# aclyde11/molecular-VAE

Measured on AMD Instinct MI355X. Metric: molecules/s (ELBO fwd+bwd+step), higher is better.
Workload: dtype bf16

## Files before the change

include/mvae.h:

```cpp
#ifndef MVAE_H_
#define MVAE_H_

#include <stddef.h>
#include <stdint.h>

#ifdef __cplusplus
extern "C" {
#endif

#define MVAE_ABI_VERSION 12

#define MVAE_OK 0
#define MVAE_ERR_INVALID (-1)
#define MVAE_ERR_WORKSPACE (-2)
#define MVAE_ERR_UNSUPPORTED (-3)

#define MVAE_F32 0
#define MVAE_BF16 1
#define MVAE_F32X3 2

#define MVAE_ACT_NONE 0
#define MVAE_ACT_SELU 1
#define MVAE_ACT_RELU 2

// ... 102 lines not shown
  int cell, dtype, layers, T, B, H;
  const void* w_hhT[MVAE_MAX_LAYERS]; int64_t ldw_hhT[MVAE_MAX_LAYERS];
  const void* w_ihT[MVAE_MAX_LAYERS]; int64_t ldw_ihT[MVAE_MAX_LAYERS];
  const int32_t* lengths;
  const float* dy; int64_t dy_ld;
  const void* dy_a; int64_t dy_a_ld; const void* dy_w; int64_t dy_w_ld; int dy_k;
  const float* dh_last[MVAE_MAX_LAYERS];
  const void* hs[MVAE_MAX_LAYERS]; int64_t ldh;
  const void* h0[MVAE_MAX_LAYERS]; int64_t ldh0;
  const void* cs[MVAE_MAX_LAYERS];
  const void* gates[MVAE_MAX_LAYERS];
  void* dG[MVAE_MAX_LAYERS]; int64_t ldg;
  void* dGh[MVAE_MAX_LAYERS];
  float* dstate[MVAE_MAX_LAYERS];
  float* dh0[MVAE_MAX_LAYERS];
  void* split_ws; size_t split_ws_bytes;
  const uint8_t* drop_mask[MVAE_MAX_LAYERS];
  float drop_p; uint32_t drop_seed;
  void* persist_ws; size_t persist_ws_bytes;
  float* poison;
  int no_spin;
} mvae_rnn_bwd_desc;

int mvae_rnn_bwd(const mvae_rnn_bwd_desc* d, void* stream, const void** status_out);
size_t mvae_rnn_bwd_persist_workspace(const mvae_rnn_bwd_desc* d);
size_t mvae_rnn_bwd_workspace(const mvae_rnn_bwd_desc* d);

int mvae_rowsum(int dtype, int R, int C, const void* X, int64_t ldx, float* out, int accumulate, void* stream);
int mvae_timesum(int dtype, int T, int B, int W, const void* X, float* out, void* stream);
size_t mvae_colsum_workspace(int M, int N);
int mvae_colsum(int M, int N, const float* X, int64_t ldx, float* out, void* ws, size_t ws_bytes, void* stream);
size_t mvae_colsum_t_workspace(int M, int N);
int mvae_colsum_t(int dtype, int M, int N, const void* X, int64_t ldx, float* out, void* ws, size_t ws_bytes, void* stream);

int mvae_conv1d_pack_weights(int Cin, int Cout, int k, const float* w , int ldx, float* wp, int ldo, float* wq,
                             void* stream);
size_t mvae_conv1d_selu_fwd_workspace(int B, int W, int ldx, int Cout, int k);
int mvae_conv1d_selu_fwd(int B, int W, int ldx, int64_t x_bs, int Cout, int k, const float* x, const float* wp, const float* bias,
                         float* y, int64_t ldy, void* ws, size_t ws_bytes, void* stream);
size_t mvae_conv1d_selu_bwd_workspace(int B, int W, int Cin, int ldx, int Cout, int ldo, int k);
int mvae_conv1d_act_fwd(int act, int B, int W, int ldx, int64_t x_bs, int Cout, int k, const float* x, const float* wp, const float* bias,
                        float* y, int64_t ldy, void* ws, size_t ws_bytes, void* stream);
#define MVAE_CONV_BWD_X3 0x100
int mvae_conv1d_act_bwd(int act, int B, int W, int Cin, int ldx, int64_t x_bs, int Cout, int ldo, int k, const float* dy, const float* y,
                        const float* x, const float* wq, float* dzp, float* dw, float* db, float* dx, int64_t lddx,
                        void* ws, size_t ws_bytes, void* stream);
int mvae_conv1d_dw_problem(int B, int W, int Cin, int ldx, int64_t x_bs, int Cout, int ldo, int k, const float* dzp, const float* x, float* dwp,
                           float* db, int x3, mvae_gemm_tn_f32_problem* out);
int mvae_conv1d_unpack_dw(int Cin, int Cout, int k, const float* dwp, int ldx, float* dw, void* stream);
int mvae_conv1d_selu_bwd(int B, int W, int Cin, int ldx, int64_t x_bs, int Cout, int ldo, int k, const float* dy, const float* y,
                         const float* x, const float* wq, float* dzp, float* dw, float* db, float* dx, int64_t lddx,
                         void* ws, size_t ws_bytes, void* stream);

int mvae_selu_bwd(int64_t n, float* dy, const float* y, void* stream);

int mvae_lambda_fwd(int B, int o, const float* mulv, const float* eps, float scale, uint32_t seed, uint64_t offset, float* eps_out,
                    float* z, float* mu, float* logvar, void* stream);
int mvae_normal_fill(int64_t n, float scale, uint32_t seed, uint64_t offset, float* out, void* stream);
void mvae_normal_words(uint32_t seed, uint64_t counter, uint32_t* words2);
int mvae_lambda_bwd(int B, int o, const float* mulv, const float* eps, const float* dz, const float* dmu,
                    const float* dlogvar, float* dmulv, void* stream);

int mvae_softmax_tb_fwd(int B, int L, int C, const float* logits, int64_t ldl, float* recon, void* stream);
int mvae_softmax_tb_bwd(int dtype, int B, int L, int C, const float* recon, const float* drecon,
                        void* dl, int64_t ldd, void* dlT, int64_t ldT, void* stream);

// ... 255 lines not shown
```

molecular-vae_amd/_lib.py:

```python
import ctypes as C
import os
import weakref

import torch

_HERE = os.path.dirname(os.path.abspath(__file__))
LIB_PATH = ((os.environ.get("MVAE_LIB") if os.environ.get("MVAE_TUNING", "0") not in ("", "0") else None)
            or os.path.join(_HERE, "libmvae_hip.so"))

ABI_VERSION = 12
MVAE_F32, MVAE_BF16, MVAE_F32X3 = 0, 1, 2
CONV_BWD_X3 = 0x100
ACT_NONE, ACT_SELU, ACT_RELU = 0, 1, 2
CELL_LSTM, CELL_GRU = 0, 1
MAX_LAYERS = 8

_vp, _i, _i64, _f, _sz, _u32 = C.c_void_p, C.c_int, C.c_int64, C.c_float, C.c_size_t, C.c_uint32


class RnnFwdDesc(C.Structure):
    _fields_ = [("cell", _i), ("dtype", _i), ("layers", _i), ("T", _i), ("B", _i), ("H", _i), ("in0", _i),
                ("x0", _vp), ("x0_ld", _i64), ("add0", _vp), ("add0_tstride", _i64),
                ("add_table", _vp), ("add_index", _vp), ("add_index_ld", _i64), ("add_table_rows", _i),
                ("w_ih", _vp * MAX_LAYERS), ("ldw_ih", _i64 * MAX_LAYERS),
# ... 59 lines not shown
    "mvae_cast_transpose": (_i, [_i, _i, _i, _i, _vp, _i64, _vp, _i64, _vp, _i64, _vp]),
    "mvae_pack_job_blocks": (_i, [C.POINTER(PackJob)]),
    "mvae_pack_multi": (_i, [_i, _vp, _i, _vp]),
    "mvae_permute021": (_i, [_i, _i, _i, _vp, _vp, _vp]),
    "mvae_gather_rows_tb": (_i, [_vp, _i, _i, _i, _vp, _i, _vp, _vp, _vp]),
    "mvae_scatter_rows_tb": (_i, [_i, _vp, _i, _i, _i, _vp, _i64, _i, _vp, _vp, _sz, _vp]),
    "mvae_scatter_rows_tb_workspace": (_sz, [_i, _i, _i, _i]),
    "mvae_onehot_tb": (_i, [_vp, _i, _i, _i, _vp, _i64, _vp]),
    "mvae_onehot_f32": (_i, [_vp, _i64, _i, _vp, _i64, _vp]),
    "mvae_rnn_fwd": (_i, [C.POINTER(RnnFwdDesc), _vp, C.POINTER(_vp)]),
    "mvae_rnn_fwd_persist_workspace": (_sz, [C.POINTER(RnnFwdDesc)]),
    "mvae_dropout_keep": (_i, [C.c_uint32, C.c_uint32, _f]),
    "mvae_gemm_tn_f32_colsum": (_i, [_i, _i, _i, _vp, _i64, _vp, _i64, _vp, _i64, _i, _vp, _i, _vp, _sz, _vp]),
    "mvae_gemm_tn_colsum_supported": (_i, [_i, _i, _i]),
    "mvae_gemm_tn_grouped_supported": (_i, [_i, _i, _i64, _i64, _i64]),
    "mvae_gemm_tn_grouped_workspace": (_sz, [_i, C.POINTER(GemmTnProblem)]),
    "mvae_gemm_tn_grouped": (_i, [_i, C.POINTER(GemmTnProblem), _vp, _sz, _vp]),
    "mvae_gemm_tn_grouped_capped": (_i, [_i, C.POINTER(GemmTnProblem), _i, _vp, _sz, _vp]),
    "mvae_gemm_tn_f32_multi_workspace": (_sz, [_i, C.POINTER(GemmTnF32Problem)]),
    "mvae_gemm_tn_f32_multi": (_i, [_i, C.POINTER(GemmTnF32Problem), _vp, _sz, _vp]),
    "mvae_conv1d_dw_problem": (_i, [_i, _i, _i, _i, _i64, _i, _i, _i, _vp, _vp, _vp, _vp, _i, C.POINTER(GemmTnF32Problem)]),
    "mvae_conv1d_unpack_dw": (_i, [_i, _i, _i, _vp, _i, _vp, _vp]),
    "mvae_gemm_tn_colsum_workspace": (_sz, [_i, _i, _i]),
    "mvae_gemm_tn_colsum": (_i, [_i, _i, _i, _vp, _i64, _vp, _i64, _vp, _i64, _i, _vp, _i, _vp, _sz, _vp]),
    "mvae_rnn_bwd": (_i, [C.POINTER(RnnBwdDesc), _vp, C.POINTER(_vp)]),
    "mvae_rnn_bwd_workspace": (_sz, [C.POINTER(RnnBwdDesc)]),
    "mvae_rnn_bwd_persist_workspace": (_sz, [C.POINTER(RnnBwdDesc)]),
    "mvae_rowsum": (_i, [_i, _i, _i, _vp, _i64, _vp, _i, _vp]),
    "mvae_timesum": (_i, [_i, _i, _i, _i, _vp, _vp, _vp]),
    "mvae_colsum_workspace": (_sz, [_i, _i]),
    "mvae_colsum": (_i, [_i, _i, _vp, _i64, _vp, _vp, _sz, _vp]),
    "mvae_colsum_t_workspace": (_sz, [_i, _i]),
    "mvae_colsum_t": (_i, [_i, _i, _i, _vp, _i64, _vp, _vp, _sz, _vp]),
    "mvae_conv1d_pack_weights": (_i, [_i, _i, _i, _vp, _i, _vp, _i, _vp, _vp]),
    "mvae_conv1d_selu_fwd_workspace": (_sz, [_i, _i, _i, _i, _i]),
    "mvae_conv1d_selu_fwd": (_i, [_i, _i, _i, _i64, _i, _i, _vp, _vp, _vp, _vp, _i64, _vp, _sz, _vp]),
    "mvae_conv1d_selu_bwd_workspace": (_sz, [_i, _i, _i, _i, _i, _i, _i]),
    "mvae_conv1d_selu_bwd": (_i, [_i, _i, _i, _i, _i64, _i, _i, _i, _vp, _vp, _vp, _vp, _vp, _vp, _vp, _vp, _i64, _vp, _sz, _vp]),
    "mvae_conv1d_act_fwd": (_i, [_i, _i, _i, _i, _i64, _i, _i, _vp, _vp, _vp, _vp, _i64, _vp, _sz, _vp]),
    "mvae_conv1d_act_bwd": (_i, [_i, _i, _i, _i, _i, _i64, _i, _i, _i, _vp, _vp, _vp, _vp, _vp, _vp, _vp, _vp, _i64, _vp, _sz, _vp]),
    "mvae_selu_bwd": (_i, [_i64, _vp, _vp, _vp]),
    "mvae_lambda_fwd": (_i, [_i, _i, _vp, _vp, _f, C.c_uint32, C.c_uint64, _vp, _vp, _vp, _vp, _vp]),
    "mvae_normal_fill": (_i, [_i64, _f, C.c_uint32, C.c_uint64, _vp, _vp]),
    "mvae_normal_words": (None, [C.c_uint32, C.c_uint64, C.POINTER(C.c_uint32)]),
    "mvae_lambda_bwd": (_i, [_i, _i, _vp, _vp, _vp, _vp, _vp, _vp, _vp]),
    "mvae_softmax_tb_fwd": (_i, [_i, _i, _i, _vp, _i64, _vp, _vp]),
    "mvae_softmax_tb_bwd": (_i, [_i, _i, _i, _i, _vp, _vp, _vp, _i64, _vp, _i64, _vp]),
    "mvae_bce_kl_loss_workspace": (_sz, [_i64, _i64]),
    "mvae_bce_kl_loss_fwd": (_i, [_i64, _vp, _vp, _i64, _vp, _vp, _f, _vp, _vp, _sz, _vp]),
    "mvae_bce_kl_loss_bwd": (_i, [_i64, _vp, _vp, _i64, _vp, _vp, _f, _vp, _vp, _vp, _vp, _vp]),
    "mvae_bce_kl_logits_workspace": (_sz, [_i, _i]),
    "mvae_bce_kl_logits_fwd": (_i, [_i, _i, _i, _vp, _i64, _vp, _i64, _vp, _vp, _f, _vp, _vp, _vp, _sz, _vp]),
    "mvae_bce_kl_logits_bwd": (_i, [_i, _i, _i, _i, _vp, _i64, _vp, _i64, _vp, _vp, _f, _vp, _vp, _i64, _vp, _i64, _vp, _vp, _vp]),
    "mvae_expand_indices": (_i, [_vp, _vp, _i, _i, _i, _vp, _vp, _vp]),
    "mvae_moses_collate": (_i, [_vp, _vp, _vp, _i, _i, _i64, _i, _i, _i, _vp, _i64, _vp, _vp, _vp, _vp]),
    "mvae_corpus_index_build": (_i, [_vp, _vp, _i64, _vp, _i64, _vp, _vp]),
    "mvae_corpus_index_probe": (_i, [_vp, _vp, _i64, _vp, _i64, _i, _i, _vp, _i64, _i, _vp, _vp]),
    "mvae_moses_latent_workspace": (_sz, [_i]),
    "mvae_moses_latent_fwd": (_i, [_i, _i, _vp, _vp, _vp, C.c_uint32, C.c_uint64, _vp, _vp, _vp, _vp, _sz, _vp]),
    "mvae_moses_latent_bwd": (_i, [_i, _i, _vp, _vp, _vp, _vp, _vp, _vp, _vp, _vp, _vp]),
    "mvae_moses_latent_fb_workspace": (_sz, [_i, _i]),
    "mvae_moses_latent_fb_fwd": (_i, [_i, _i, _vp, _vp, _vp, C.c_uint32, C.c_uint64, _vp, _f, _vp, _vp, _vp, _vp, _sz, _vp]),
    "mvae_moses_latent_fb_bwd": (_i, [_i, _i, _vp, _vp, _vp, _vp, _vp, _vp, _vp, _f, _vp, _vp, _vp]),
    "mvae_token_dropout": (_i, [_vp, _vp, _i, _i, _i, _f, C.c_uint32, _vp, _vp, _vp, _vp]),
    "mvae_ce_loss_workspace": (_sz, [_i, _i]),
    "mvae_ce_loss_fwd": (_i, [_i, _i, _i, _vp, _i64, _vp, _i, _vp, _vp, _sz, _vp]),
# ... 182 lines not shown
```

molecular-vae_amd/csrc/elementwise.hip:

```cpp
#include "common.hpp"
#include "kernels.hpp"
#include <stdlib.h>

static inline int grid_for(long n, int per_block = 256, int cap = 2048) {
  long b = (n + per_block - 1) / per_block;
  if (b < 1) b = 1;
  if (b > cap) b = cap;
  return (int)b;
}

template <typename TS, typename TD>
__global__ __launch_bounds__(256) void cast_transpose_kernel(int R, int C, const TS* src, long lds_, TD* dst, long ldd, TD* dstT, long ldt) {
  __shared__ float tile[32][33];
  const int c0 = blockIdx.x * 32, r0 = blockIdx.y * 32;
  const int tx = threadIdx.x & 31, ty = threadIdx.x >> 5;
#pragma unroll
  for (int i = 0; i < 4; ++i) {
    const int r = r0 + ty + i * 8, c = c0 + tx;
    float v = 0.f;
    if (r < R && c < C) v = TT<TS>::ld(src + (long)r * lds_ + c);
    tile[ty + i * 8][tx] = v;
    if (dst && r < R && c < ldd) TT<TD>::st(dst + (long)r * ldd + c, v);
  }
  if (!dstT) return;
// ... 89 lines not shown
__global__ __launch_bounds__(256) void scatter_rows_tb_stage1(const int64_t* idx, int B, int L, int nrows, const T* d, long ldd, int W,
                                                              int rpb, int ws_cols, float* partial) {
  extern __shared__ __attribute__((aligned(16))) char smem_raw[];
  float* tab = reinterpret_cast<float*>(smem_raw);
  const long total = (long)B * L;
  const int c_lo = blockIdx.y * ws_cols;
  int c_hi = c_lo + ws_cols; if (c_hi > W) c_hi = W;
  const int wsl = c_hi - c_lo;
  for (int i = threadIdx.x; i < nrows * ws_cols; i += 256) tab[i] = 0.f;
  __syncthreads();
  const long rbeg = (long)blockIdx.x * rpb;
  long rend = rbeg + rpb; if (rend > total) rend = total;
  for (int c = threadIdx.x; c < wsl; c += 256) {
    for (long row0 = rbeg; row0 < rend; row0 += 8) {
      float v[8]; int id[8];
#pragma unroll
      for (int r = 0; r < 8; ++r) {
        const long row = row0 + r;
        if (row < rend) {
          const int t = (int)(row / B), b = (int)(row - (long)t * B);
          long q = idx[(long)b * L + t];
          id[r] = (int)(q < 0 ? 0 : (q >= nrows ? nrows - 1 : q));
          v[r] = TT<T>::ld(d + row * ldd + c_lo + c);
        } else { id[r] = 0; v[r] = 0.f; }
      }
#pragma unroll
      for (int r = 0; r < 8; ++r) tab[id[r] * ws_cols + c] += v[r];
    }
  }
  __syncthreads();
  float* out = partial + (long)blockIdx.x * nrows * W;
  for (int i = threadIdx.x; i < nrows * wsl; i += 256) { const int r = i / wsl, c = i - r * wsl; out[(long)r * W + c_lo + c] = tab[r * ws_cols + c]; }
}
__global__ __launch_bounds__(256) void sum_partials_kernel(const float* partial, int nparts, long n, float* out) {
  __shared__ float red[4][64];
  const int e = threadIdx.x & 63, slot = threadIdx.x >> 6;
  const long i = (long)blockIdx.x * 64 + e;
  float v = 0.f;
  if (i < n) for (int k = slot; k < nparts; k += 4) v += partial[(long)k * n + i];
  red[slot][e] = v;
  __syncthreads();
  if (slot == 0 && i < n) out[i] = (red[0][e] + red[1][e]) + (red[2][e] + red[3][e]);
}

__global__ __launch_bounds__(256) void permute021_kernel(int N, int A, int Bd, const float* in, float* out) {
  const long n = (long)N * A * Bd;
  for (long i = (long)blockIdx.x * 256 + threadIdx.x; i < n; i += (long)gridDim.x * 256) {
    const int a = (int)(i % A); const long nb = i / A; const int b = (int)(nb % Bd); const long nn = nb / Bd;
    out[i] = in[(nn * A + a) * Bd + b];
  }
}

__global__ __launch_bounds__(256) void selu_bwd_kernel(long n, float* dy, const float* y) {
  for (long i = (long)blockIdx.x * 256 + threadIdx.x; i < n; i += (long)gridDim.x * 256) dy[i] *= selu_grad_from_out(y[i]);
}
int launch_selu_bwd(long n, float* dy, const float* y, hipStream_t st) {
  if (n <= 0) return MVAE_OK;
  hipLaunchKernelGGL(selu_bwd_kernel, dim3(grid_for(n)), dim3(256), 0, st, n, dy, y);
  MVAE_CHECK_HIP(hipGetLastError());
  return MVAE_OK;
}

__global__ __launch_bounds__(256) void colsum_stage1_kernel(int M, int N, const float* X, long ldx, int rows_per_chunk, float* partial) {
  __shared__ float red[4][64];
  const int c = blockIdx.x * 64 + (threadIdx.x & 63), g = threadIdx.x >> 6;
  const int r0 = blockIdx.y * rows_per_chunk;
// ... 38 lines not shown
    for (int m = r0 + rs; m < r1; m += 8) {
      float v[8];
      const T* p = X + (long)m * ldx + c0;
      if (n == 8) {
        if constexpr (sizeof(T) == 2) {
          const uint4 u = *reinterpret_cast<const uint4*>(p);
          const uint32_t w[4] = {u.x, u.y, u.z, u.w};
#pragma unroll
          for (int i = 0; i < 4; ++i) { v[2 * i] = __builtin_bit_cast(float, w[i] << 16); v[2 * i + 1] = __builtin_bit_cast(float, w[i] & 0xffff0000u); }
        } else {
          const float4 x0 = *reinterpret_cast<const float4*>(p), x1 = *reinterpret_cast<const float4*>(p + 4);
          v[0] = x0.x; v[1] = x0.y; v[2] = x0.z; v[3] = x0.w; v[4] = x1.x; v[5] = x1.y; v[6] = x1.z; v[7] = x1.w;
        }
      } else {
#pragma unroll
        for (int e = 0; e < 8; ++e) v[e] = (e < n) ? TT<T>::ld(p + e) : 0.f;
      }
#pragma unroll
      for (int e = 0; e < 8; ++e) a[e] += v[e];
    }
  }
#pragma unroll
  for (int e = 0; e < 8; ++e) red[rs][cg * 8 + e] = a[e];
  __syncthreads();
  const int c = blockIdx.x * 256 + threadIdx.x;
  if (c < N) {
    float v = 0.f;
#pragma unroll
    for (int k = 0; k < 8; ++k) v += red[k][threadIdx.x];
    partial[(long)blockIdx.y * N + c] = v;
  }
}
static int colsum_t_chunks(int M) { int c = (M + 511) / 512; if (c > 64) c = 64; if (c < 1) c = 1; return c; }

template <typename T> __device__ __forceinline__ float sum_chunk16(const uint4& v);
template <> __device__ __forceinline__ float sum_chunk16<float>(const uint4& v) {
  return (__builtin_bit_cast(float, v.x) + __builtin_bit_cast(float, v.y)) + (__builtin_bit_cast(float, v.z) + __builtin_bit_cast(float, v.w));
}
template <> __device__ __forceinline__ float sum_chunk16<bf16_t>(const uint4& v) {
  float a = 0.f;
  const uint32_t w[4] = {v.x, v.y, v.z, v.w};
#pragma unroll
  for (int i = 0; i < 4; ++i) a += __builtin_bit_cast(float, w[i] << 16) + __builtin_bit_cast(float, w[i] & 0xffff0000u);
  return a;
}
template <typename T>
__global__ __launch_bounds__(256) void rowsum_kernel(int R, int C, const T* X, long ldx, float* out, int accumulate) {
  constexpr int EPC = TT<T>::EPC;
  const int r = blockIdx.x * 4 + (threadIdx.x >> 6), lane = threadIdx.x & 63;
  if (r >= R) return;
  const T* p = X + (long)r * ldx;
  float v = 0.f;
  int c0 = 0;
  if ((reinterpret_cast<uintptr_t>(p) & 15) == 0) {
    const int nch = C / EPC;
    for (int i = lane; i < nch; i += 64) v += sum_chunk16<T>(*reinterpret_cast<const uint4*>(p + (long)i * EPC));
    c0 = nch * EPC;
  }
  for (int c = c0 + lane; c < C; c += 64) v += TT<T>::ld(p + c);
  v = wave_sum(v);
  if (lane == 0) out[r] = accumulate ? out[r] + v : v;
}
template <typename T>
__global__ __launch_bounds__(256) void timesum_kernel(int T_, long BW, const T* X, float* out) {
  for (long i = (long)blockIdx.x * 256 + threadIdx.x; i < BW; i += (long)gridDim.x * 256) {
    float v = 0.f;
// ... 1012 lines not shown
}

int mvae_pack_job_blocks(const mvae_pack_job* j) {
  if (!j || j->R < 1 || j->C < 1) return 0;
  if (j->kind == 1) return (int)(((long)j->R * j->C + 1023) / 1024);
  return ((j->C + 31) / 32) * ((j->R + 31) / 32);
}
int mvae_pack_multi(int njobs, const mvae_pack_job* jobs_device, int total_blocks, void* stream) {
  if (njobs < 1 || !jobs_device || total_blocks < 1) return MVAE_ERR_INVALID;
  hipLaunchKernelGGL(pack_multi_kernel, dim3((unsigned)total_blocks), dim3(256), 0, (hipStream_t)stream, njobs, jobs_device);
  MVAE_CHECK_HIP(hipGetLastError());
  return MVAE_OK;
}

int mvae_permute021(int N, int A, int Bd, const float* in, float* out, void* stream) {
  if (!in || !out || N < 1 || A < 1 || Bd < 1) return MVAE_ERR_INVALID;
  hipLaunchKernelGGL(permute021_kernel, dim3(grid_for((long)N * A * Bd)), dim3(256), 0, (hipStream_t)stream, N, A, Bd, in, out);
  MVAE_CHECK_HIP(hipGetLastError());
  return MVAE_OK;
}

int mvae_gather_rows_tb(const int64_t* idx, int B, int L, int nrows, const float* table, int W, const float* base, float* out, void* stream) {
  if (!idx || !table || !out || B < 1 || L < 1 || W < 1 || nrows < 1) return MVAE_ERR_INVALID;
  hipLaunchKernelGGL(gather_rows_tb_kernel, dim3(grid_for((long)B * L * W)), dim3(256), 0, (hipStream_t)stream, idx, B, L, nrows, table, W, base, out);
  MVAE_CHECK_HIP(hipGetLastError());
  return MVAE_OK;
}

static int scatter_parts(int B, int L) { long rows = (long)B * L; long parts = (rows + 63) / 64; if (parts > 1024) parts = 1024; return (int)parts; }
size_t mvae_scatter_rows_tb_workspace(int B, int L, int nrows, int W) { return (size_t)scatter_parts(B, L) * nrows * W * sizeof(float); }
int mvae_scatter_rows_tb(int dtype, const int64_t* idx, int B, int L, int nrows, const void* d, int64_t ldd, int W, float* dtable,
                         void* ws, size_t ws_bytes, void* stream) {
  if (!idx || !d || !dtable || B < 1 || L < 1 || W < 1 || nrows < 1) return MVAE_ERR_INVALID;
  int ws_cols = (48 * 1024) / (nrows * (int)sizeof(float));
  if (ws_cols < 1) return MVAE_ERR_UNSUPPORTED;
  if (ws_cols > W) ws_cols = W;
  const int slices = (W + ws_cols - 1) / ws_cols;
  const size_t ldsb = (size_t)nrows * ws_cols * sizeof(float);
  const int parts = scatter_parts(B, L);
  if (!ws || ws_bytes < mvae_scatter_rows_tb_workspace(B, L, nrows, W)) return MVAE_ERR_WORKSPACE;
  const long rows = (long)B * L;
  const int rpb = (int)((rows + parts - 1) / parts);
  hipStream_t st = (hipStream_t)stream;
  if (dtype == MVAE_F32)
    hipLaunchKernelGGL((scatter_rows_tb_stage1<float>), dim3(parts, slices), dim3(256), ldsb, st, idx, B, L, nrows, (const float*)d, ldd, W, rpb, ws_cols, (float*)ws);
  else if (dtype == MVAE_BF16)
    hipLaunchKernelGGL((scatter_rows_tb_stage1<bf16_t>), dim3(parts, slices), dim3(256), ldsb, st, idx, B, L, nrows, (const bf16_t*)d, ldd, W, rpb, ws_cols, (float*)ws);
  else return MVAE_ERR_INVALID;
  hipLaunchKernelGGL(sum_partials_kernel, dim3((unsigned)(((long)nrows * W + 63) / 64)), dim3(256), 0, st, (const float*)ws, parts, (long)nrows * W, dtable);
  MVAE_CHECK_HIP(hipGetLastError());
  return MVAE_OK;
}

int mvae_rowsum(int dtype, int R, int C, const void* X, int64_t ldx, float* out, int accumulate, void* stream) {
  if (!X || !out || R < 1) return MVAE_ERR_INVALID;
  hipStream_t st = (hipStream_t)stream;
  if (dtype == MVAE_F32) hipLaunchKernelGGL((rowsum_kernel<float>), dim3((R + 3) / 4), dim3(256), 0, st, R, C, (const float*)X, ldx, out, accumulate);
  else if (dtype == MVAE_BF16) hipLaunchKernelGGL((rowsum_kernel<bf16_t>), dim3((R + 3) / 4), dim3(256), 0, st, R, C, (const bf16_t*)X, ldx, out, accumulate);
  else return MVAE_ERR_INVALID;
  MVAE_CHECK_HIP(hipGetLastError());
  return MVAE_OK;
}
int mvae_timesum(int dtype, int T, int B, int W, const void* X, float* out, void* stream) {
  if (!X || !out || T < 1 || B < 1 || W < 1) return MVAE_ERR_INVALID;
  hipStream_t st = (hipStream_t)stream;
  const long BW = (long)B * W;
// ... 2 lines not shown
    if (BW % 8 == 0 && ((reinterpret_cast<uintptr_t>(X) | reinterpret_cast<uintptr_t>(out)) & 15) == 0)
      hipLaunchKernelGGL(timesum_bf16x8_kernel, dim3(grid_for(BW / 8, 256, 8192)), dim3(256), 0, st, T, BW, (const bf16_t*)X, out);
    else hipLaunchKernelGGL((timesum_kernel<bf16_t>), dim3(grid_for(BW, 256, 8192)), dim3(256), 0, st, T, BW, (const bf16_t*)X, out);
  } else return MVAE_ERR_INVALID;
  MVAE_CHECK_HIP(hipGetLastError());
  return MVAE_OK;
}
int mvae_onehot_f32(const int64_t* idx, int64_t n, int nrows, float* out, int64_t ld, void* stream) {
  if (!idx || !out || n < 1 || nrows < 1 || ld < nrows || (ld % 4) || (reinterpret_cast<uintptr_t>(out) & 15)) return MVAE_ERR_INVALID;
  hipLaunchKernelGGL(onehot_f32_kernel, dim3(grid_for((long)n * (ld / 4))), dim3(256), 0, (hipStream_t)stream, idx, (long)n, nrows, out, (long)ld);
  MVAE_CHECK_HIP(hipGetLastError());
  return MVAE_OK;
}
int mvae_onehot_tb(const int64_t* idx, int B, int L, int nrows, void* out, int64_t ld, void* stream) {
  if (!idx || !out || B < 1 || L < 1 || nrows < 1 || ld < nrows || (ld % 8) || (reinterpret_cast<uintptr_t>(out) & 15)) return MVAE_ERR_INVALID;
  hipLaunchKernelGGL(onehot_tb_kernel, dim3(grid_for((long)B * L * (ld / 8))), dim3(256), 0, (hipStream_t)stream, idx, B, L, nrows,
                     reinterpret_cast<bf16_t*>(out), (long)ld);
  MVAE_CHECK_HIP(hipGetLastError());
  return MVAE_OK;
}
size_t mvae_colsum_t_workspace(int M, int N) { return (size_t)colsum_t_chunks(M) * N * sizeof(float); }
int mvae_colsum_t(int dtype, int M, int N, const void* X, int64_t ldx, float* out, void* ws, size_t ws_bytes, void* stream) {
  if (!X || !out || M < 0 || N < 1) return MVAE_ERR_INVALID;
  if ((ldx % 8) || (reinterpret_cast<uintptr_t>(X) & 15)) return MVAE_ERR_INVALID;
  if (!ws || ws_bytes < mvae_colsum_t_workspace(M, N)) return MVAE_ERR_WORKSPACE;
  hipStream_t st = (hipStream_t)stream;
  const int chunks = colsum_t_chunks(M);
  const int rpc = (M + chunks - 1) / chunks;
  dim3 grid((N + 255) / 256, chunks);
  if (dtype == MVAE_F32) hipLaunchKernelGGL((colsum_t_stage1_kernel<float>), grid, dim3(256), 0, st, M, N, (const float*)X, ldx, rpc, (float*)ws);
  else if (dtype == MVAE_BF16) hipLaunchKernelGGL((colsum_t_stage1_kernel<bf16_t>), grid, dim3(256), 0, st, M, N, (const bf16_t*)X, ldx, rpc, (float*)ws);
  else return MVAE_ERR_INVALID;
  hipLaunchKernelGGL(sum_partials_kernel, dim3((unsigned)((N + 63) / 64)), dim3(256), 0, st, (const float*)ws, chunks, (long)N, out);
  MVAE_CHECK_HIP(hipGetLastError());
  return MVAE_OK;
}
size_t mvae_colsum_workspace(int M, int N) { return colsum_workspace_bytes(M, N); }
int mvae_colsum(int M, int N, const float* X, int64_t ldx, float* out, void* ws, size_t ws_bytes, void* stream) {
  if (!X || !out || M < 0) return MVAE_ERR_INVALID;
  return launch_colsum(M, N, X, ldx, out, ws, ws_bytes, (hipStream_t)stream);
}
int mvae_expand_indices(const uint8_t* store, const int64_t* rows, int B, int L, int C, int64_t* idx, float* ohe, void* stream) {
  if (!store || !rows || !idx || B < 1 || L < 1 || C < 1) return MVAE_ERR_INVALID;
  hipLaunchKernelGGL(expand_indices_kernel, dim3(grid_for((long)B * L)), dim3(256), 0, (hipStream_t)stream, store, rows, B, L, C, idx, ohe);
  MVAE_CHECK_HIP(hipGetLastError());
  return MVAE_OK;
}
int mvae_moses_collate(const uint8_t* tokens, const int64_t* offsets, const int64_t* rows, int B, int T, int64_t N, int bos, int eos, int pad,
                       int64_t* x_pad, int64_t x_ld, int32_t* lengths, int64_t* rows_sorted, int32_t* err, void* stream) {
  if (!tokens || !offsets || !rows || !x_pad || !lengths || B < 1 || T < 2 || N < 1 || x_ld < T) return MVAE_ERR_INVALID;
  if (bos < 0 || bos > 65535 || eos < 0 || eos > 65535 || pad < 0 || pad > 65535) return MVAE_ERR_INVALID;
  hipLaunchKernelGGL(moses_collate_kernel, dim3((B + 3) / 4), dim3(256), 0, (hipStream_t)stream, tokens, offsets, rows, B, T, (long)N, bos, eos, pad,
                     x_pad, (long)x_ld, lengths, rows_sorted, err);
  MVAE_CHECK_HIP(hipGetLastError());
  return MVAE_OK;
}
int mvae_relu_bwd(int64_t n, float* dy, const float* y, void* stream) {
  if (!dy || !y) return MVAE_ERR_INVALID;
  if (n <= 0) return MVAE_OK;
  hipLaunchKernelGGL(relu_bwd_kernel, dim3(grid_for(n)), dim3(256), 0, (hipStream_t)stream, (long)n, dy, y);
  MVAE_CHECK_HIP(hipGetLastError());
  return MVAE_OK;
}
int mvae_permute102(int T, int B, int V, const float* in, float* out, void* stream) {
  if (!in || !out || T < 1 || B < 1 || V < 1) return MVAE_ERR_INVALID;
  hipLaunchKernelGGL(permute102_kernel, dim3(grid_for((long)T * B * V)), dim3(256), 0, (hipStream_t)stream, T, B, V, in, out);
// ... 323 lines not shown
```

molecular-vae_amd/models.py:

```python
import math
import os
import weakref

import torch
import torch.nn as nn

from . import _lib as L
from . import ops


def _pad(n, m):
    return (n + m - 1) // m * m


class _NoCompute(nn.Module):
    def forward(self, *a, **k):
        raise RuntimeError(f"{type(self).__name__} only holds parameters; the arithmetic runs in the fused HIP path "
                           "of the enclosing MolEncoder / MolDecoder")


def _holder_forward(*a, **k):
    raise RuntimeError("this nn.Linear only holds parameters; the arithmetic runs in the fused HIP path of the enclosing module")


# ... 761 lines not shown
    gates = [W(f"gates{l}", (Lq, B, G4), dt) for l in range(NL)]
    fuse_ok = dt == torch.bfloat16 and (4 * H) % 64 == 0
    use_pb = fuse_ok and ops.rnn_bwd_persist_wanted(L.CELL_LSTM, dt, NL, B, H, ldg, dev)
    fuse_dy = fuse_ok and not use_pb
    ldl = _dyk(Cv) if fuse_ok else Cp
    dl = W("dl", (TB + 8, ldl), dt)[:TB]
    dlT = None
    if dt != torch.bfloat16:
        ldT = _pad(TB, 8) + 8
        dlT = W("dlT", (Cv, ldT), dt)
    fill_dl(ws, dl, dlT)
    dy = None
    if not fuse_dy:
        dy = W("dy", (TB, H))
        ops.gemm_nt(dl, P["WoutT"], dy, TB, H, ldl if fuse_ok else Cp)
    dG = [W(f"dG{l}", (Lq, B, ldg), dt) for l in range(NL)]
    dstate = [W(f"dstate{l}", (2, B, H)) for l in range(NL)]
    ops.rnn_bwd(L.CELL_LSTM, dt, Lq, B, H, P["WhhT"], [P["ldwT"]] * NL, P["WihT"], [P["ldwT"]] * NL, dy, H, hs, ldh, cs, gates,
                dG, dstate, ldg=ldg, tag="dec_lstm_bwd", dy_a=(dl if fuse_dy else None), dy_w=(P["WoutT"] if fuse_dy else None),
                dy_k=(_dyk(Cv) if fuse_dy else 0), poison=L.grad_poison(params))

    gsync = getattr(sink[0], "grad_sync", None) if sink is not None else None
    dp_early = gsync is not None and gsync.active and gsync.allow_early
    late_all = TB <= WGRAD_LATE_TB
    nlow = 0 if late_all else min(2, NL - 1)
    if dp_early:
        parts = [[l] for l in range(NL - 1, -1, -1)]
    else:
        parts = [list(range(nlow, NL))] + ([list(range(nlow))] if nlow >= 1 else [])
    first_name = lambda l: f"gru.weight_ih_l{l}" if l >= 1 else "gru.weight_hh_l0"

    wg_cap = [0]

    def weight_grads(k):
        with ops._Timed("dec_lstm_wgrad" if (k is None or k == 0) else "dec_lstm_wgrad_deferred"):
            if k is None or k == 0:
                if dt == torch.bfloat16:
                    ops.gemm_tn(dl, hs[-1].view(TB, ldh), grads["decoded_mean.module.0.weight"], Cv, H, TB, lda=ldl, ldb=ldh)
                    dbp = W("dbout_p", (Cp,))
                    ops.colsum_t(dl, TB, Cp, dbp, ldx=ldl)
                    grads["decoded_mean.module.0.bias"].copy_(dbp[:Cv])
                else:
                    hsT = W("wg_hsT_out", (H, ldT), dt)
                    ops.cast_transpose(hs[-1].view(TB, ldh), TB, H, dstT=hsT, lds=ldh)
                    ops.gemm_nt(dlT, hsT, grads["decoded_mean.module.0.weight"], Cv, H, TB, lda=ldT, ldb=ldT)
                    ops.rowsum(dlT, Cv, TB, grads["decoded_mean.module.0.bias"])
            layers = range(NL) if k is None else parts[k]
            _lstm_weight_grads(ws, grads, "gru", dt, dev, NL, Lq, B, H, dG, ldg, hs, ldh, layers=layers, max_workgroups=wg_cap[0])
            if k is not None and dp_early:
                lo = sink[2] + offs[first_name(min(parts[k]))]
                hi = sink[3] if k == 0 else sink[2] + offs[first_name(min(parts[k - 1]))]
                gsync.start_early(sink[1], lo, hi)

    peer = mod.__dict__["_peer"]() if mod.__dict__["_peer"] is not None else None
    fork = bool(mod.overlap_weight_grads and peer is not None and ctx.from_peer and ctx.needs_input_grad[1] and
                all(p.grad is None for p in params))
    if fork:
        side = mod._side_stream(dev)
        gflat.record_stream(side)
        fstate = peer.__dict__["_fork"]
        if late_all:
            wg_cap[0] = WGRAD_CAP
            for k in range(len(parts)):
                fstate.park(side, (lambda kk=k: weight_grads(kk)), -1)
            fstate.run_deferred(stage=-1)
        else:
            for k in range(len(parts)):
                fstate.park(side, (lambda kk=k: weight_grads(kk)), 1 if 2 * k >= len(parts) else 0)
    else:
        weight_grads(None)
    dgx0 = W("dgx0", (B, ldg))
    ops.timesum(dG[0], Lq, B, ldg, dgx0)
    li = W("li", (B, o))
    ops.gemm_tn(dgx0, li, grads["gru.weight_ih_l0"], G4, o, B, lda=ldg)
    dli = W("dli", (B, o))
    ops.gemm_nt(dgx0, P["Wih0T"], dli, B, o, G4)
    ops.selu_bwd(dli, li)
    ops.gemm_tn_f32_colsum(dli, z, grads["latent_input.0.weight"], grads["latent_input.0.bias"], o, o, B)
    dz = torch.empty(B, o, dtype=f32, device=dev)
    ops.gemm_nt(dli, P["WliT"], dz, B, o, o, ldb=P["WliT"].stride(0))
    if fork:
        for n, p in zip(names, params):
            p.grad = grads[n]
        return dz, (None,) * len(names)
    return dz, tuple(grads[n] for n in names)


class _DecoderFn(torch.autograd.Function):
    @staticmethod
    @ops.traced("molvae_decoder_fwd")
    def forward(ctx, mod, z, infer, *params):
        z, logits = _decoder_fwd_logits(ctx, mod, z, infer, params)
        B, Lq, Cv = z.shape[0], mod.repeat_vector.rep, mod.decoded_mean.module[0].out_features
        recon = torch.empty(B, Lq, Cv, dtype=torch.float32, device=z.device)
        with ops._Timed("hbm_softmax_fwd"):
            ops.softmax_tb_fwd(logits, Cv, recon, B, Lq, Cv)
        ctx.save_for_backward(recon)
        return recon

    @staticmethod
    @ops.traced("molvae_decoder_bwd")
# ... 97 lines not shown
```

molecular-vae_amd/ops.py:

```python
import ctypes as C
import weakref

import torch

from . import _lib as L
from ._lib import ptr, check, stream_ptr, dt_code


def _pad(n, m):
    return (n + m - 1) // m * m


PROFILE = None


_ROCTX = {"lib": None, "on": None}


def enable_roctx(on=True):
    if on and _ROCTX["lib"] is None:
        for name in ("libroctx64.so", "librocprofiler-sdk-roctx.so", "/opt/rocm/lib/libroctx64.so"):
            try:
                lib = C.CDLL(name)
                lib.roctxRangePushA.argtypes = [C.c_char_p]
# ... 255 lines not shown
        q.C, q.ldc, q.accumulate = out.data_ptr(), (out.stride(0) if ldc is None else ldc), 1 if accumulate else 0
        q.colsum_out = colsum_out.data_ptr() if colsum_out is not None else None
        q.colsum_accumulate, q.x3 = (1 if colsum_accumulate else 0), (1 if x3 else 0)
        self.probs.append(q)
        self.keep += [A, B, out, colsum_out]

    def add_conv_dw(self, B, W, Cin, ldx, x_bs, Cout, ldo, k, dzp, x, dwp, dw, db, x3=False):
        q = L.GemmTnF32Problem()
        check(L.load().mvae_conv1d_dw_problem(B, W, Cin, ldx, x_bs, Cout, ldo, k, ptr(dzp), ptr(x), ptr(dwp), ptr(db), 1 if x3 else 0, C.byref(q)),
              "mvae_conv1d_dw_problem")
        self.probs.append(q)
        self.keep += [dzp, x, dwp, db, dw]
        self.after.append(lambda: check(L.load().mvae_conv1d_unpack_dw(Cin, Cout, k, ptr(dwp), ldx, ptr(dw), stream_ptr()), "mvae_conv1d_unpack_dw"))

    def run(self):
        lib = L.load()
        for i in range(0, len(self.probs), self.MAX):
            part = self.probs[i:i + self.MAX]
            arr = (L.GemmTnF32Problem * len(part))(*part)
            need = lib.mvae_gemm_tn_f32_multi_workspace(len(part), arr)
            ws = Scratch.get(need, self.device, tag="tn_f32_multi") if need else None
            check(lib.mvae_gemm_tn_f32_multi(len(part), arr, ptr(ws), need, stream_ptr()), "mvae_gemm_tn_f32_multi")
        for fn in self.after:
            fn()
        self.probs, self.keep, self.after = [], [], []


def colsum_t(X, M, N, out, ldx=None):
    lib = L.load()
    need = lib.mvae_colsum_t_workspace(M, N)
    ws = Scratch.get(need, X.device)
    check(lib.mvae_colsum_t(dt_code(X.dtype), M, N, ptr(X), X.stride(0) if ldx is None else ldx, ptr(out), ptr(ws), need,
                            stream_ptr()), "mvae_colsum_t")


def cast_transpose(src, R, C_, dst=None, dstT=None, lds=None):
    lib = L.load()
    lds = src.stride(0) if lds is None else lds
    d = dst if dst is not None else dstT
    check(lib.mvae_cast_transpose(dt_code(src.dtype), dt_code(d.dtype), R, C_, ptr(src), lds,
                                  ptr(dst), dst.stride(0) if dst is not None else 0,
                                  ptr(dstT), dstT.stride(0) if dstT is not None else 0, stream_ptr()), "mvae_cast_transpose")


class PackList:

    def __init__(self):
        self.jobs, self.keep, self.table, self.total = [], [], None, 0

    def _job(self, kind, src, R, C_, lds, dst=None, ldd=0, dstT=None, ldt=0, src2=None, dst_dtype=None):
        j = L.PackJob()
        j.kind, j.R, j.C = kind, R, C_
        j.src_dtype = dt_code(src.dtype)
        d = dst if dst is not None else dstT
        j.dst_dtype = dt_code(d.dtype if dst_dtype is None else dst_dtype)
        j.src, j.lds = src.data_ptr(), lds
        j.dst, j.ldd = (dst.data_ptr() if dst is not None else None), ldd
        j.dstT, j.ldt = (dstT.data_ptr() if dstT is not None else None), ldt
        j.src2 = src2.data_ptr() if src2 is not None else None
        self.jobs.append(j)
        self.keep += [t for t in (src, dst, dstT, src2) if t is not None]
        self.table = None

    def cast_transpose(self, src, R, C_, dst=None, dstT=None, lds=None):
        if R <= 0 or C_ <= 0:
            return
# ... 1128 lines not shown
```

Before: 38030.

## Add narrow colsum and LDS scatter kernels, split head grads onto side stream

Adds a narrow-column colsum kernel for the bf16 decoder output bias gradient, so the padded colsum_t plus copy is skipped when the vocabulary width is at most 256. Adds an LDS-resident scatter_rows_tb path for f32 when the whole table fits in shared memory, followed by a wide partial-sum reduction. The output head weight and bias gradients are now parked as their own early deferred job on the side stream, so they run ahead of the LSTM weight-grad parts. This is meant to cut reduction overhead and improve overlap, at the cost of extra workspace and more kernel variants.

```diff
diff --git a/include/mvae.h b/include/mvae.h
--- a/include/mvae.h
+++ b/include/mvae.h
@@ -158,6 +158,8 @@
 int mvae_colsum(int M, int N, const float* X, int64_t ldx, float* out, void* ws, size_t ws_bytes, void* stream);
 size_t mvae_colsum_t_workspace(int M, int N);
 int mvae_colsum_t(int dtype, int M, int N, const void* X, int64_t ldx, float* out, void* ws, size_t ws_bytes, void* stream);
+size_t mvae_colsum_narrow_workspace(int M, int N);
+int mvae_colsum_narrow(int dtype, int M, int N, const void* X, int64_t ldx, float* out, void* ws, size_t ws_bytes, void* stream);
 
 int mvae_conv1d_pack_weights(int Cin, int Cout, int k, const float* w , int ldx, float* wp, int ldo, float* wq,
                              void* stream);
diff --git a/molecular-vae_amd/_lib.py b/molecular-vae_amd/_lib.py
--- a/molecular-vae_amd/_lib.py
+++ b/molecular-vae_amd/_lib.py
@@ -115,6 +115,8 @@
     "mvae_colsum": (_i, [_i, _i, _vp, _i64, _vp, _vp, _sz, _vp]),
     "mvae_colsum_t_workspace": (_sz, [_i, _i]),
     "mvae_colsum_t": (_i, [_i, _i, _i, _vp, _i64, _vp, _vp, _sz, _vp]),
+    "mvae_colsum_narrow_workspace": (_sz, [_i, _i]),
+    "mvae_colsum_narrow": (_i, [_i, _i, _i, _vp, _i64, _vp, _vp, _sz, _vp]),
     "mvae_conv1d_pack_weights": (_i, [_i, _i, _i, _vp, _i, _vp, _i, _vp, _vp]),
     "mvae_conv1d_selu_fwd_workspace": (_sz, [_i, _i, _i, _i, _i]),
     "mvae_conv1d_selu_fwd": (_i, [_i, _i, _i, _i64, _i, _i, _vp, _vp, _vp, _vp, _i64, _vp, _sz, _vp]),
diff --git a/molecular-vae_amd/csrc/elementwise.hip b/molecular-vae_amd/csrc/elementwise.hip
--- a/molecular-vae_amd/csrc/elementwise.hip
+++ b/molecular-vae_amd/csrc/elementwise.hip
@@ -145,6 +145,56 @@
   float* out = partial + (long)blockIdx.x * nrows * W;
   for (int i = threadIdx.x; i < nrows * wsl; i += 256) { const int r = i / wsl, c = i - r * wsl; out[(long)r * W + c_lo + c] = tab[r * ws_cols + c]; }
 }
+constexpr int SCATTER_TILE = 256;
+constexpr size_t SCATTER_LDS_MAX = 80 * 1024;
+__global__ __launch_bounds__(1024) void scatter_rows_tb_lds_kernel(const int64_t* idx, int B, int L, int nrows, const float* d, long ldd, int W,
+                                                                   int rpb, float* partial) {
+  extern __shared__ __attribute__((aligned(16))) char smem_raw[];
+  float* tab = reinterpret_cast<float*>(smem_raw);
+  int* ids = reinterpret_cast<int*>(tab + nrows * W);
+  const int nt = blockDim.x, c = threadIdx.x;
+  for (int i = c; i < nrows * W; i += nt) tab[i] = 0.f;
+  const long total = (long)B * L;
+  const long rbeg = (long)blockIdx.x * rpb;
+  long rend = rbeg + rpb; if (rend > total) rend = total;
+  for (long t0 = rbeg; t0 < rend; t0 += SCATTER_TILE) {
+    __syncthreads();
+    const int n = rend - t0 < SCATTER_TILE ? (int)(rend - t0) : SCATTER_TILE;
+    for (int i = c; i < SCATTER_TILE; i += nt) {
+      int off = 0;
+      if (i < n) {
+        const long row = t0 + i;
+        const int t = (int)(row / B), b = (int)(row - (long)t * B);
+        const long q = idx[(long)b * L + t];
+        off = (int)(q < 0 ? 0 : (q >= nrows ? nrows - 1 : q)) * W;
+      }
+      ids[i] = off;
+    }
+    __syncthreads();
+    if (c < W) {
+      const float* p = d + t0 * ldd + c;
+      auto load = [&](float (&v)[16], int i) {
+#pragma unroll
+        for (int r = 0; r < 16; ++r) { const float x = p[(long)(i + r < n ? i + r : n - 1) * ldd]; v[r] = i + r < n ? x : 0.f; }
+      };
+      auto apply = [&](const float (&v)[16], int i) {
+#pragma unroll
+        for (int r = 0; r < 16; ++r) tab[ids[i + r] + c] += v[r];
+      };
+      float va[16], vb[16];
+      load(va, 0);
+      for (int i = 0; i < n; i += 32) {
+        load(vb, i + 16);
+        apply(va, i);
+        load(va, i + 32);
+        if (i + 16 < n) apply(vb, i + 16);
+      }
+    }
+  }
+  __syncthreads();
+  float* out = partial + (long)blockIdx.x * nrows * W;
+  for (int i = c; i < nrows * W; i += nt) out[i] = tab[i];
+}
 __global__ __launch_bounds__(256) void sum_partials_kernel(const float* partial, int nparts, long n, float* out) {
   __shared__ float red[4][64];
   const int e = threadIdx.x & 63, slot = threadIdx.x >> 6;
@@ -249,6 +299,72 @@
   }
 }
 static int colsum_t_chunks(int M) { int c = (M + 511) / 512; if (c > 64) c = 64; if (c < 1) c = 1; return c; }
+
+template <int E>
+__global__ __launch_bounds__(1024) void sum_partials_wide_kernel(const float* partial, int nparts, long n, float* out) {
+  constexpr int S = 1024 / E;
+  __shared__ float red[S][E + 1];
+  const int e = threadIdx.x % E, slot = threadIdx.x / E;
+  const long i = (long)blockIdx.x * E + e;
+  float v = 0.f;
+  if (i < n) {
+#pragma unroll 8
+    for (int k = slot; k < nparts; k += S) v += partial[(long)k * n + i];
+  }
+  red[slot][e] = v;
+  __syncthreads();
+  if (slot == 0 && i < n) {
+    float s = 0.f;
+#pragma unroll
+    for (int k = 0; k < S; ++k) s += red[k][e];
+    out[i] = s;
+  }
+}
+
+template <typename T>
+__global__ __launch_bounds__(256) void colsum_narrow_stage1_kernel(int M, int N, const T* X, long ldx, int rows_per_chunk, float* partial) {
+  constexpr int EPC = TT<T>::EPC;
+  __shared__ float red[256][EPC + 1];
+  const int ncg = (N + EPC - 1) / EPC, rpp = 256 / ncg;
+  const int rs = threadIdx.x / ncg, cg = threadIdx.x - rs * ncg;
+  const long r0 = (long)blockIdx.x * rows_per_chunk;
+  long r1 = r0 + rows_per_chunk; if (r1 > M) r1 = M;
+  float a[EPC];
+#pragma unroll
+  for (int e = 0; e < EPC; ++e) a[e] = 0.f;
+  if (rs < rpp) {
+    const T* p = X + cg * EPC;
+    for (long m = r0 + rs; m < r1; m += 4L * rpp) {
+      uint4 u[4];
+#pragma unroll
+      for (int k = 0; k < 4; ++k) {
+        const long r = m + (long)k * rpp;
+        u[k] = r < r1 ? *reinterpret_cast<const uint4*>(p + r * ldx) : make_uint4(0u, 0u, 0u, 0u);
+      }
+#pragma unroll
+      for (int k = 0; k < 4; ++k) {
+        const uint32_t w[4] = {u[k].x, u[k].y, u[k].z, u[k].w};
+        if constexpr (sizeof(T) == 2) {
+#pragma unroll
+          for (int i = 0; i < 4; ++i) { a[2 * i] += __builtin_bit_cast(float, w[i] << 16); a[2 * i + 1] += __builtin_bit_cast(float, w[i] & 0xffff0000u); }
+        } else {
+#pragma unroll
+          for (int i = 0; i < 4; ++i) a[i] += __builtin_bit_cast(float, w[i]);
+        }
+      }
+    }
+  }
+#pragma unroll
+  for (int e = 0; e < EPC; ++e) red[threadIdx.x][e] = a[e];
+  __syncthreads();
+  if ((int)threadIdx.x < N) {
+    const int g = threadIdx.x / EPC, e = threadIdx.x - g * EPC;
+    float v = 0.f;
+    for (int k = 0; k < rpp; ++k) v += red[k * ncg + g][e];
+    partial[(long)blockIdx.x * N + threadIdx.x] = v;
+  }
+}
+static int colsum_narrow_chunks(int M) { int c = (M + 63) / 64; if (c > 1024) c = 1024; if (c < 1) c = 1; return c; }
 
 template <typename T> __device__ __forceinline__ float sum_chunk16(const uint4& v);
 template <> __device__ __forceinline__ float sum_chunk16<float>(const uint4& v) {
@@ -1327,6 +1443,23 @@
 int mvae_scatter_rows_tb(int dtype, const int64_t* idx, int B, int L, int nrows, const void* d, int64_t ldd, int W, float* dtable,
                          void* ws, size_t ws_bytes, void* stream) {
   if (!idx || !d || !dtable || B < 1 || L < 1 || W < 1 || nrows < 1) return MVAE_ERR_INVALID;
+  const size_t lds_whole = (size_t)nrows * W * sizeof(float) + SCATTER_TILE * sizeof(int);
+  if (dtype == MVAE_F32 && W <= 1024 && lds_whole <= SCATTER_LDS_MAX) {
+    const long rows = (long)B * L;
+    long parts = (rows + 63) / 64; if (parts > 512) parts = 512;
+    if (!ws || ws_bytes < (size_t)parts * nrows * W * sizeof(float)) return MVAE_ERR_WORKSPACE;
+    const int rpb = (int)((rows + parts - 1) / parts);
+    hipStream_t st = (hipStream_t)stream;
+    static bool attr_set = false;
+    if (!attr_set) {
+      MVAE_CHECK_HIP(hipFuncSetAttribute(reinterpret_cast<const void*>(scatter_rows_tb_lds_kernel), hipFuncAttributeMaxDynamicSharedMemorySize, (int)SCATTER_LDS_MAX));
+      attr_set = true;
+    }
+    hipLaunchKernelGGL(scatter_rows_tb_lds_kernel, dim3((unsigned)parts), dim3((W + 63) / 64 * 64), lds_whole, st, idx, B, L, nrows, (const float*)d, ldd, W, rpb, (float*)ws);
+    hipLaunchKernelGGL((sum_partials_wide_kernel<64>), dim3((unsigned)(((long)nrows * W + 63) / 64)), dim3(1024), 0, st, (const float*)ws, (int)parts, (long)nrows * W, dtable);
+    MVAE_CHECK_HIP(hipGetLastError());
+    return MVAE_OK;
+  }
   int ws_cols = (48 * 1024) / (nrows * (int)sizeof(float));
   if (ws_cols < 1) return MVAE_ERR_UNSUPPORTED;
   if (ws_cols > W) ws_cols = W;
@@ -1395,6 +1528,22 @@
   else if (dtype == MVAE_BF16) hipLaunchKernelGGL((colsum_t_stage1_kernel<bf16_t>), grid, dim3(256), 0, st, M, N, (const bf16_t*)X, ldx, rpc, (float*)ws);
   else return MVAE_ERR_INVALID;
   hipLaunchKernelGGL(sum_partials_kernel, dim3((unsigned)((N + 63) / 64)), dim3(256), 0, st, (const float*)ws, chunks, (long)N, out);
+  MVAE_CHECK_HIP(hipGetLastError());
+  return MVAE_OK;
+}
+size_t mvae_colsum_narrow_workspace(int M, int N) { return (size_t)colsum_narrow_chunks(M) * (N > 0 ? N : 0) * sizeof(float); }
+int mvae_colsum_narrow(int dtype, int M, int N, const void* X, int64_t ldx, float* out, void* ws, size_t ws_bytes, void* stream) {
+  if (!X || !out || M < 0 || N < 1) return MVAE_ERR_INVALID;
+  if (N > 256) return MVAE_ERR_UNSUPPORTED;
+  if (ldx < N || (ldx % 8) || (reinterpret_cast<uintptr_t>(X) & 15)) return MVAE_ERR_INVALID;
+  if (!ws || ws_bytes < mvae_colsum_narrow_workspace(M, N)) return MVAE_ERR_WORKSPACE;
+  hipStream_t st = (hipStream_t)stream;
+  const int chunks = colsum_narrow_chunks(M);
+  const int rpc = (M + chunks - 1) / chunks;
+  if (dtype == MVAE_F32) hipLaunchKernelGGL((colsum_narrow_stage1_kernel<float>), dim3(chunks), dim3(256), 0, st, M, N, (const float*)X, ldx, rpc, (float*)ws);
+  else if (dtype == MVAE_BF16) hipLaunchKernelGGL((colsum_narrow_stage1_kernel<bf16_t>), dim3(chunks), dim3(256), 0, st, M, N, (const bf16_t*)X, ldx, rpc, (float*)ws);
+  else return MVAE_ERR_INVALID;
+  hipLaunchKernelGGL((sum_partials_wide_kernel<16>), dim3((unsigned)((N + 15) / 16)), dim3(1024), 0, st, (const float*)ws, chunks, (long)N, out);
   MVAE_CHECK_HIP(hipGetLastError());
   return MVAE_OK;
 }
diff --git a/molecular-vae_amd/models.py b/molecular-vae_amd/models.py
--- a/molecular-vae_amd/models.py
+++ b/molecular-vae_amd/models.py
@@ -817,19 +817,25 @@
 
     wg_cap = [0]
 
-    def weight_grads(k):
+    def head_grads():
+        if dt == torch.bfloat16:
+            ops.gemm_tn(dl, hs[-1].view(TB, ldh), grads["decoded_mean.module.0.weight"], Cv, H, TB, lda=ldl, ldb=ldh)
+            if Cv <= 256 and not late_all:
+                ops.colsum_narrow(dl, TB, Cv, grads["decoded_mean.module.0.bias"], ldx=ldl)
+            else:
+                dbp = W("dbout_p", (Cp,))
+                ops.colsum_t(dl, TB, Cp, dbp, ldx=ldl)
+                grads["decoded_mean.module.0.bias"].copy_(dbp[:Cv])
+        else:
+            hsT = W("wg_hsT_out", (H, ldT), dt)
+            ops.cast_transpose(hs[-1].view(TB, ldh), TB, H, dstT=hsT, lds=ldh)
+            ops.gemm_nt(dlT, hsT, grads["decoded_mean.module.0.weight"], Cv, H, TB, lda=ldT, ldb=ldT)
+            ops.rowsum(dlT, Cv, TB, grads["decoded_mean.module.0.bias"])
+
+    def weight_grads(k, head=True):
         with ops._Timed("dec_lstm_wgrad" if (k is None or k == 0) else "dec_lstm_wgrad_deferred"):
-            if k is None or k == 0:
-                if dt == torch.bfloat16:
-                    ops.gemm_tn(dl, hs[-1].view(TB, ldh), grads["decoded_mean.module.0.weight"], Cv, H, TB, lda=ldl, ldb=ldh)
-                    dbp = W("dbout_p", (Cp,))
-                    ops.colsum_t(dl, TB, Cp, dbp, ldx=ldl)
-                    grads["decoded_mean.module.0.bias"].copy_(dbp[:Cv])
-                else:
-                    hsT = W("wg_hsT_out", (H, ldT), dt)
-                    ops.cast_transpose(hs[-1].view(TB, ldh), TB, H, dstT=hsT, lds=ldh)
-                    ops.gemm_nt(dlT, hsT, grads["decoded_mean.module.0.weight"], Cv, H, TB, lda=ldT, ldb=ldT)
-                    ops.rowsum(dlT, Cv, TB, grads["decoded_mean.module.0.bias"])
+            if head and (k is None or k == 0):
+                head_grads()
             layers = range(NL) if k is None else parts[k]
             _lstm_weight_grads(ws, grads, "gru", dt, dev, NL, Lq, B, H, dG, ldg, hs, ldh, layers=layers, max_workgroups=wg_cap[0])
             if k is not None and dp_early:
@@ -850,8 +856,10 @@
                 fstate.park(side, (lambda kk=k: weight_grads(kk)), -1)
             fstate.run_deferred(stage=-1)
         else:
+            fstate.park(side, head_grads, -1)
+            fstate.run_deferred(stage=-1)
             for k in range(len(parts)):
-                fstate.park(side, (lambda kk=k: weight_grads(kk)), 1 if 2 * k >= len(parts) else 0)
+                fstate.park(side, (lambda kk=k: weight_grads(kk, head=False)), 1 if 2 * k >= len(parts) else 0)
     else:
         weight_grads(None)
     dgx0 = W("dgx0", (B, ldg))
diff --git a/molecular-vae_amd/ops.py b/molecular-vae_amd/ops.py
--- a/molecular-vae_amd/ops.py
+++ b/molecular-vae_amd/ops.py
@@ -311,6 +311,14 @@
     ws = Scratch.get(need, X.device)
     check(lib.mvae_colsum_t(dt_code(X.dtype), M, N, ptr(X), X.stride(0) if ldx is None else ldx, ptr(out), ptr(ws), need,
                             stream_ptr()), "mvae_colsum_t")
+
+
+def colsum_narrow(X, M, N, out, ldx=None):
+    lib = L.load()
+    need = lib.mvae_colsum_narrow_workspace(M, N)
+    ws = Scratch.get(need, X.device)
+    check(lib.mvae_colsum_narrow(dt_code(X.dtype), M, N, ptr(X), X.stride(0) if ldx is None else ldx, ptr(out), ptr(ws), need,
+                                 stream_ptr()), "mvae_colsum_narrow")
 
 
 def cast_transpose(src, R, C_, dst=None, dstT=None, lds=None):
```

Result: no change. 38280, median of 6 (+0.7%).
